# NVlabs/CenterPose

Hardware: NVIDIA H100
Metric: images/sec at 512x512 DLA-34 (dla_34 + DCNv2, 7 heads, decode + PnP) (higher is better)
Workload: dtype tf32x3

## Files before the change

centerpose_b200/csrc/conv_tma.cu:

```cuda
#include <cuda.h>

#include "common.cuh"
#include "umma_common.cuh"

namespace cp {
namespace {

constexpr int TM_BM = 128;
constexpr int TM_THREADS = 384;
constexpr int TM_THREADS_X3 = 512;

struct TmaConvParams {
  CUtensorMap amap[4];
  int nsrc;
  int srcC[4];
  int B, H, W, Cin, Cout, CoutPad, BN;
  int k;
  int tile_m;
  int Wt, boxh;
  int tiles_per_image;
  long long total_tiles;
  long long m_tiles;
  uint32_t slab_bytes, slab_stride;
  int SA, SB;
// ... 156 lines not shown
          if constexpr (MULTI) {
            const TileGeo g = decode_tile<MULTI>(p, tile / KS_SPLIT, n_tiles);
            wsrc = p.wtiles + (size_t)g.model * p.tstride +
                   ((size_t)g.n_tile * KB_all + (size_t)(tile % KS_SPLIT) * KB) * btile_bytes;
          } else {
            const int n_tile = (int)((tile / KS_SPLIT) % n_tiles);
            wsrc = p.wtiles + ((size_t)n_tile * KB_all + (size_t)(tile % KS_SPLIT) * KB) * btile_bytes;
          }
          for (int kb = 0; kb < KB; ++kb) {
            mbar_wait(smem_u32(&ctl->b_empty[stage]), phase ^ 1u);
            const uint32_t bar = smem_u32(&ctl->b_full[stage]);
            mbar_arrive_expect_tx(bar, btile_bytes);
            bulk_g2s(btiles0 + (uint32_t)stage * btile_bytes, wsrc + (size_t)kb * btile_bytes, btile_bytes, bar);
            if (++stage == p.SB) {
              stage = 0;
              phase ^= 1u;
            }
          }
        }
      }
      __syncwarp();
    }
  } else if (X3 && warp >= 12) {
    asm volatile("setmaxnreg.dec.sync.aligned.u32 48;");
    const int st = tid - 384;
    int stage = 0;
    uint32_t phase = 0;
    const uint32_t nchunk = p.slab_bytes >> 4;
    for (long long it = 0, tile = tile_at(0); tile < total_tiles; tile = tile_at(++it)) {
      for (int s = 0; s < sps; ++s) {
        mbar_wait(smem_u32(&ctl->a_full[stage]), phase);
        const uint32_t hi = slabs0 + (uint32_t)stage * a_stage;
        const uint32_t lo = hi + p.slab_stride;
        for (uint32_t c0 = st; c0 < nchunk; c0 += 128 * 4) {
          float4 v[4];
#pragma unroll
          for (int u = 0; u < 4; ++u)
            if (c0 + u * 128 < nchunk) v[u] = ld_shared_v4f(hi + ((c0 + u * 128) << 4));
#pragma unroll
          for (int u = 0; u < 4; ++u) {
            if (c0 + u * 128 < nchunk) {
              float4 h, l;
              h.x = tf32_round(v[u].x); l.x = tf32_round(v[u].x - h.x);
              h.y = tf32_round(v[u].y); l.y = tf32_round(v[u].y - h.y);
              h.z = tf32_round(v[u].z); l.z = tf32_round(v[u].z - h.z);
              h.w = tf32_round(v[u].w); l.w = tf32_round(v[u].w - h.w);
              st_shared_v4f(hi + ((c0 + u * 128) << 4), h.x, h.y, h.z, h.w);
              st_shared_v4f(lo + ((c0 + u * 128) << 4), l.x, l.y, l.z, l.w);
            }
          }
        }
        fence_proxy_async_smem();
        mbar_arrive(smem_u32(&ctl->a_split[stage]));
        if (++stage == p.SA) {
          stage = 0;
          phase ^= 1u;
        }
      }
    }
  } else {
    if (X3) asm volatile("setmaxnreg.inc.sync.aligned.u32 208;");
    const int c = (warp - 4) >> 2, wt = tid & 127;
    float* dstage = reinterpret_cast<float*>(smem + (drain0 - smem_u32(smem))) + (size_t)c * (DRAIN_STAGE_BYTES / 4);
    const uint32_t bar_a = smem_u32(X3 ? &ctl->a_split[0] : &ctl->a_full[0]);
    const uint32_t bar_a_empty = smem_u32(&ctl->a_empty[0]);
    const uint32_t bar_b_full = smem_u32(&ctl->b_full[0]), bar_b_empty = smem_u32(&ctl->b_empty[0]);
    const uint32_t a_lo_u = p.slab_stride >> 4, b_lo_u = ((uint32_t)BN * rowb) >> 4;
    EpiParams ep;
    ep.bias = p.bias;
    ep.residual = p.residual;
    ep.resStride = p.resStride;
    ep.relu = p.relu;
    ep.res_after_relu = p.res_after_relu;
    ep.round_tf32 = p.round_tf32;
    ep.out = p.out;
    ep.outStride = p.outStride;
    ep.out_nchw = p.out_nchw;
    ep.Cout = p.Cout;
    ep.CoutPad = p.CoutPad;
    ep.H = p.H;
    ep.W = p.W;
    int sa = 0, sb = 0;
    uint32_t pa = 0, pb = 0;
    float acc[BN / 2];
    float sums[X3 ? BN / 2 : 1];
    float acc2[FUSE ? 16 : 1];
#pragma unroll
    for (int j = 0; j < BN / 2; ++j) acc[j] = 0.f;
#pragma unroll
    for (int j = 0; j < (FUSE ? 16 : 1); ++j) acc2[j] = 0.f;
    for (long long it = 0, tile = tile_at(0); tile < total_tiles; tile = tile_at(++it)) {
      const TileGeo g = decode_tile<MULTI>(p, tile / KS_SPLIT, n_tiles);
      const uint32_t row0 = (p.k == 3 ? (uint32_t)(g.g0 - 1 - g.r_lo * p.Wt) : 0u) + (uint32_t)c * 64u;
#pragma unroll
      for (int j = 0; j < (X3 ? BN / 2 : 1); ++j) sums[j] = 0.f;
      int kbi = 0, gk = 0;
      for (int s = 0; s < sps; ++s) {
        mbar_wait(bar_a + 8u * (uint32_t)sa, pa);
        const uint32_t a_slab = slabs0 + (uint32_t)sa * a_stage;
        for (int tap = 0; tap < taps; ++tap, ++kbi) {
          const int ky = tap / 3, kx = tap - ky * 3;
          const uint32_t arow = row0 + (p.k == 3 ? (uint32_t)(ky * p.Wt + kx) : 0u);
          mbar_wait(bar_b_full + 8u * (uint32_t)sb, pb);
          const uint64_t da = make_desc(a_slab + arow * rowb, p.cslab);
          const uint64_t db = make_desc(btiles0 + (uint32_t)sb * btile_bytes, p.cslab);
          const bool fresh = X3 ? gk == 0 : kbi == 0;
          if (p.cslab == 32)
            mma_kblock<BN, X3, false, 4>(acc, da, db, a_lo_u, b_lo_u, fresh);
          else
            mma_kblock<BN, X3, false, 2>(acc, da, db, a_lo_u, b_lo_u, fresh);
          if (wt == 0) {
            mbar_arrive(bar_b_empty + 8u * (uint32_t)sb);
            if (tap == taps - 1) mbar_arrive(bar_a_empty + 8u * (uint32_t)sa);
          }
          if (++sb == p.SB) {
            sb = 0;
            pb ^= 1u;
          }
          if (X3) {
            if (gk == p.group - 1 || kbi == KB - 1) {
#pragma unroll
              for (int j = 0; j < (X3 ? BN / 2 : 1); ++j) sums[j] += acc[X3 ? j : 0];
              gk = 0;
            } else {
              ++gk;
            }
          }
        }
        if (++sa == p.SA) {
          sa = 0;
          pa ^= 1u;
        }
      }
      const int r_me = wt >> 1;
      int n, oy, ox, m;
      const bool valid = tile_position<MULTI>(p, g, c * 64 + r_me, &n, &oy, &ox, &m);
      const int col_end = min(p.Cout, (g.n_tile + 1) * BN);
      const int head = FUSE ? g.n_tile / p.tph : 0, part = FUSE ? g.n_tile - head * p.tph : 0;
      const size_t wofs = MULTI ? (size_t)g.model * p.wstride : 0;
      if (MULTI) ep.bias = p.bias + wofs;
      if (FUSE && part == 0) {
#pragma unroll
        for (int j = 0; j < (FUSE ? 16 : 1); ++j) acc2[j] = 0.f;
      }
      auto fn = [&](int r, int cb, float (&v)[16]) {
        if (cb >= BN) return;
        if (!FUSE && KS_SPLIT > 1) {
          const long long mn = tile / KS_SPLIT;
          const int ks = (int)(tile % KS_SPLIT);
          float4* mine = reinterpret_cast<float4*>(p.part) + (((size_t)mn * KS_SPLIT + ks) * (BN >> 2) + (cb >> 2)) * p.tile_m +
                         c * 64 + r;
#pragma unroll
          for (int q = 0; q < 4; ++q) __stcg(mine + (size_t)q * p.tile_m, make_float4(v[4 * q], v[4 * q + 1], v[4 * q + 2], v[4 * q + 3]));
        } else if (FUSE) {
          const float* b1 = p.bias + wofs + (size_t)g.n_tile * BN + cb;
          const float4* w2 = reinterpret_cast<const float4*>(p.fuse_w[head] + wofs) + ((size_t)part * BN + cb) * 4;
#pragma unroll
          for (int q = 0; q < 16; ++q) {
            const float h = fmaxf(v[q] + __ldg(b1 + q), 0.f);
#pragma unroll
            for (int u = 0; u < 4; ++u) {
              const float4 w = __ldg(w2 + q * 4 + u);
              acc2[FUSE ? 4 * u + 0 : 0] = fmaf(h, w.x, acc2[FUSE ? 4 * u + 0 : 0]);
              acc2[FUSE ? 4 * u + 1 : 0] = fmaf(h, w.y, acc2[FUSE ? 4 * u + 1 : 0]);
              acc2[FUSE ? 4 * u + 2 : 0] = fmaf(h, w.z, acc2[FUSE ? 4 * u + 2 : 0]);
              acc2[FUSE ? 4 * u + 3 : 0] = fmaf(h, w.w, acc2[FUSE ? 4 * u + 3 : 0]);
            }
          }
        } else {
          epilogue_row<16>(ep, v, valid, m, n, oy, ox, g.n_tile * BN + cb, col_end);
        }
      };
      if constexpr (X3)
        drain_rows<BN>(sums, dstage, wt, 1 + c, fn);
      else
        drain_rows<BN>(acc, dstage, wt, 1 + c, fn);
      if (FUSE && part == p.tph - 1) {
#pragma unroll
        for (int j = 0; j < (FUSE ? 16 : 1); ++j) acc2[j] += __shfl_xor_sync(0xffffffffu, acc2[j], 1);
        if ((wt & 1) == 0 && valid) {
          const int co = p.fuse_cout[head];
          float* o = p.fuse_out[head] + ((size_t)n * co * p.H + oy) * p.W + ox;
          const size_t plane = (size_t)p.H * p.W;
#pragma unroll
          for (int j = 0; j < 16; ++j)
            if (j < co) o[j * plane] = acc2[FUSE ? j : 0] + __ldg(p.fuse_b[head] + wofs + j);
        }
      }
    }
  }
}

__global__ void pack_tma_weight_kernel(const float* __restrict__ src, int ld, int Cin, int taps, int Cout, int BN, int n_tiles,
                                       int round_tf32, int x3, int cslab, unsigned char* __restrict__ dst) {
  const int KB = (Cin / cslab) * taps;
  const int cpr = cslab / 4;
  const size_t rowb = (size_t)cslab * 4;
  const size_t total = (size_t)n_tiles * KB * BN * cpr;
  for (size_t i = blockIdx.x * (size_t)blockDim.x + threadIdx.x; i < total; i += (size_t)gridDim.x * blockDim.x) {
    const int q = i % cpr;
    size_t t = i / cpr;
    const int nr = t % BN;
    t /= BN;
    const int kb = t % KB;
    const int nt = t / KB;
    const int n = nt * BN + nr;
    const int slab = kb / taps, tap = kb - slab * taps;
    float v[4];
#pragma unroll
    for (int j = 0; j < 4; ++j) {
      const int k = tap * Cin + slab * cslab + q * 4 + j;
      float x = (n < Cout) ? src[(size_t)k * ld + n] : 0.f;
      v[j] = round_tf32 ? tf32_round(x) : x;
    }
    const size_t tile = ((size_t)nt * KB + kb) * (size_t)BN * rowb * (x3 ? 2 : 1);
    const int sw = cslab == 32 ? (nr & 7) : ((nr >> 1) & 3);
    const size_t off = (size_t)nr * rowb + (size_t)((q ^ sw) << 4);
    *reinterpret_cast<float4*>(dst + tile + off) = make_float4(v[0], v[1], v[2], v[3]);
    if (x3) {
      float l[4];
#pragma unroll
      for (int j = 0; j < 4; ++j) {
        const int k = tap * Cin + slab * cslab + q * 4 + j;
        const float x = (n < Cout) ? src[(size_t)k * ld + n] : 0.f;
        l[j] = tf32_round(x - v[j]);
      }
      *reinterpret_cast<float4*>(dst + tile + (size_t)BN * rowb + off) = make_float4(l[0], l[1], l[2], l[3]);
    }
  }
}

typedef CUresult (*EncodeTiledFn)(CUtensorMap*, CUtensorMapDataType, cuuint32_t, void*, const cuuint64_t*, const cuuint64_t*,
                                  const cuuint32_t*, const cuuint32_t*, CUtensorMapInterleave, CUtensorMapSwizzle,
                                  CUtensorMapL2promotion, CUtensorMapFloatOOBfill);

EncodeTiledFn get_encode() {
  static EncodeTiledFn fn = nullptr;
  if (!fn) {
    void* p = nullptr;
    cudaDriverEntryPointQueryResult q;
    if (cudaGetDriverEntryPoint("cuTensorMapEncodeTiled", &p, cudaEnableDefault, &q) == cudaSuccess &&
        q == cudaDriverEntryPointSuccess)
      fn = (EncodeTiledFn)p;
  }
  return fn;
}

}

template <bool MULTI>
__global__ void __launch_bounds__(256) conv_tma_splitk_finish(const __grid_constant__ TmaConvParams p, long long mn_tiles) {
  splitk_finish<MULTI>(p, p.tile_m, mn_tiles, [&](long long mn, int i, int* n, int* oy, int* ox) {
    int m;
    return tile_position<MULTI>(p, decode_tile<MULTI>(p, mn, p.CoutPad / p.BN), i, n, oy, ox, &m);
  });
}

static int tma_boxh(int Wt) { return (TM_BM + 1 + 2 * Wt + Wt - 1) / Wt + 1; }

// ... 35 lines not shown
  if (p.mode != IGEMM_NHWC_VEC) return false;
  if (!((p.kh == 1 && p.kw == 1 && p.pad == 0) || (p.kh == 3 && p.kw == 3 && p.pad == 1))) return false;
  if (p.stride != 1) return false;
  const int cs = tma_cslab(p, x3);
  if (p.Cin % cs) return false;
  for (int s = 0; s < p.nsrc; ++s)
    if (p.srcC[s] % cs || p.srcStride[s] % 4) return false;
  if (p.kh == 3 && p.Win + 2 > 256) return false;
  const int bn = tma_tile_n(p.CoutPad, x3);
  if (bn == 0) return false;
  const size_t slab = p.kh == 3 ? (size_t)tma_boxh(p.Win + 2) * (p.Win + 2) * cs * 4 : (size_t)TM_BM * cs * 4;
  const size_t a_stage = ((slab + 1023) / 1024 * 1024) * (x3 ? 2 : 1);
  const size_t btile = (size_t)bn * cs * 4 * (x3 ? 2 : 1);
  if (a_stage + 2 * btile > TM_BUDGET) return false;
  return get_encode() != nullptr;
}

size_t tma_weight_bytes(int Cin, int taps, int CoutPad, int x3) {
  return (size_t)CoutPad * Cin * taps * 4 * (x3 ? 2 : 1);
}

int launch_pack_tma_weight(const float* src, int ld, int Cin, int taps, int Cout, int CoutPad, int x3, int cs, int bn,
                           void* dst, cudaStream_t s) {
  const int nt = CoutPad / bn;
  size_t total = (size_t)nt * (Cin / cs) * taps * bn * (cs / 4);
  int blocks = (int)((total + 255) / 256);
  if (blocks > 132 * 32) blocks = 132 * 32;
  pack_tma_weight_kernel<<<blocks, 256, 0, s>>>(src, ld, Cin, taps, Cout, bn, nt, 1, x3, cs, (unsigned char*)dst);
  CP_LAUNCH_CHECK("pack_tma_weight_kernel");
  return CP_OK;
}

int tma_encode_nhwc_box(const float* base, int C, int W, int H, int B, int strideFloats, int boxC, int boxW, int boxH,
                        int swizzle64, void* map_out) {
  EncodeTiledFn enc = get_encode();
  if (!enc) return fail(CP_ERR_CUDA, "cuTensorMapEncodeTiled entry point not available");
  cuuint64_t dims[4] = {(cuuint64_t)C, (cuuint64_t)W, (cuuint64_t)H, (cuuint64_t)B};
  cuuint64_t strides[3] = {(cuuint64_t)strideFloats * 4, (cuuint64_t)W * strideFloats * 4, (cuuint64_t)H * W * strideFloats * 4};
  cuuint32_t box[4] = {(cuuint32_t)boxC, (cuuint32_t)boxW, (cuuint32_t)boxH, 1};
  cuuint32_t es[4] = {1, 1, 1, 1};
  CUresult r = enc(reinterpret_cast<CUtensorMap*>(map_out), CU_TENSOR_MAP_DATA_TYPE_FLOAT32, 4, (void*)base, dims, strides, box,
                   es, CU_TENSOR_MAP_INTERLEAVE_NONE, swizzle64 ? CU_TENSOR_MAP_SWIZZLE_64B : CU_TENSOR_MAP_SWIZZLE_NONE,
                   CU_TENSOR_MAP_L2_PROMOTION_L2_256B,
                   CU_TENSOR_MAP_FLOAT_OOB_FILL_NONE);
  if (r != CUDA_SUCCESS) return fail(CP_ERR_CUDA, "cuTensorMapEncodeTiled failed with code " + std::to_string((int)r));
  return CP_OK;
}

int tma_conv_encode(const IgemmParams& p, int Bmax, int cs, void* maps_out) {
  EncodeTiledFn enc = get_encode();
  if (!enc) return fail(CP_ERR_CUDA, "cuTensorMapEncodeTiled entry point not available");
  CUtensorMap* maps = reinterpret_cast<CUtensorMap*>(maps_out);
  const int Wt = p.Win + 2;
  const int boxh = tma_boxh(Wt);
  const CUtensorMapSwizzle swz = cs == 32 ? CU_TENSOR_MAP_SWIZZLE_128B : CU_TENSOR_MAP_SWIZZLE_64B;
  for (int s = 0; s < p.nsrc; ++s) {
    CUresult r;
    if (p.kh == 3) {
      cuuint64_t dims[4] = {(cuuint64_t)p.srcC[s], (cuuint64_t)p.Win, (cuuint64_t)p.Hin, (cuuint64_t)Bmax};
      cuuint64_t strides[3] = {(cuuint64_t)p.srcStride[s] * 4, (cuuint64_t)p.Win * p.srcStride[s] * 4,
                               (cuuint64_t)p.Hin * p.Win * p.srcStride[s] * 4};
      cuuint32_t box[4] = {(cuuint32_t)cs, (cuuint32_t)Wt, (cuuint32_t)boxh, 1};
      cuuint32_t es[4] = {1, 1, 1, 1};
      r = enc(&maps[s], CU_TENSOR_MAP_DATA_TYPE_FLOAT32, 4, (void*)p.src[s], dims, strides, box, es,
              CU_TENSOR_MAP_INTERLEAVE_NONE, swz, CU_TENSOR_MAP_L2_PROMOTION_L2_256B,
              CU_TENSOR_MAP_FLOAT_OOB_FILL_NONE);
    } else {
      cuuint64_t dims[2] = {(cuuint64_t)p.srcC[s], (cuuint64_t)Bmax * p.Hin * p.Win};
      cuuint64_t strides[1] = {(cuuint64_t)p.srcStride[s] * 4};
      cuuint32_t box[2] = {(cuuint32_t)cs, (cuuint32_t)TM_BM};
      cuuint32_t es[2] = {1, 1};
      r = enc(&maps[s], CU_TENSOR_MAP_DATA_TYPE_FLOAT32, 2, (void*)p.src[s], dims, strides, box, es,
              CU_TENSOR_MAP_INTERLEAVE_NONE, swz, CU_TENSOR_MAP_L2_PROMOTION_L2_256B,
              CU_TENSOR_MAP_FLOAT_OOB_FILL_NONE);
    }
    if (r != CUDA_SUCCESS) return fail(CP_ERR_CUDA, "cuTensorMapEncodeTiled failed with code " + std::to_string((int)r));
  }
  return CP_OK;
}

template <bool X3, bool FUSE, bool MULTI>
static int launch_conv_tma_kernel(const TmaConvParams& q, const cudaLaunchConfig_t& cfg0) {
  void (*kern)(TmaConvParams) = nullptr;
  switch (q.BN) {
    case 16: kern = conv_tma_kernel<X3, FUSE, 16, MULTI>; break;
    case 32: kern = conv_tma_kernel<X3, FUSE, 32, MULTI>; break;
    case 64: kern = conv_tma_kernel<X3, FUSE, 64, MULTI>; break;
    case 128: kern = conv_tma_kernel<X3, FUSE, 128, MULTI>; break;
    default: return fail(CP_ERR_INVALID, "conv_tma: unsupported N tile");
  }
  static PerDevice<bool, 4> configured;
  const int slot = q.BN == 128 ? 3 : (q.BN == 64 ? 2 : (q.BN == 32 ? 1 : 0));
  if (!configured.here(slot)) {
    CP_CUDA_CHECK(cudaFuncSetAttribute(kern, cudaFuncAttributeMaxDynamicSharedMemorySize, 227 * 1024));
    configured.here(slot) = true;
  }
  cudaLaunchConfig_t cfg = cfg0;
  cudaLaunchAttribute attr[1];
  attr[0].id = cudaLaunchAttributeProgrammaticStreamSerialization;
  attr[0].val.programmaticStreamSerializationAllowed = 1;
  cfg.attrs = attr;
  cfg.numAttrs = g_pdl ? 1 : 0;
  CP_CUDA_CHECK(cudaLaunchKernelEx(&cfg, kern, q));
  CP_LAUNCH_CHECK("conv_tma_kernel");
  return CP_OK;
}

int launch_conv_tma(const IgemmParams& p, const void* maps, const ConvKernel& k, cudaStream_t stream, LaunchInfo* info) {
  if (!p.wgt_umma) return fail(CP_ERR_INVALID, "conv_tma: weight tiles missing");
  if (p.B % model_ipm(p)) return fail(CP_ERR_INVALID, "conv_tma: batch is not a whole number of models");
  const bool x3 = k.x3;
  TmaConvParams q;
  memset(&q, 0, sizeof(q));
  memcpy(q.amap, maps, sizeof(CUtensorMap) * 4);
  q.nsrc = p.nsrc;
  for (int s = 0; s < 4; ++s) q.srcC[s] = p.srcC[s];
  q.B = p.B;
  q.H = p.Hin;
  q.W = p.Win;
  q.Cin = p.Cin;
  q.Cout = p.Cout;
  q.CoutPad = p.CoutPad;
  q.BN = k.BN;
  q.x3 = x3;
  q.cslab = k.cslab;
  q.group = kX3GroupBlocks * (32 / q.cslab);
  q.k = p.kh;
  q.Wt = p.Win + 2;
  q.tile_m = TM_BM;
  q.boxh = tma_boxh(q.Wt);
  q.ipm = model_ipm(p);
  q.wstride = p.wstride;
  q.tstride = p.tstride;
  size_t m_tiles;
  if (q.k == 3) {
    q.tiles_per_image = (p.Hin * q.Wt + q.tile_m - 1) / q.tile_m;
    m_tiles = (size_t)q.tiles_per_image * p.B;
    q.slab_bytes = (uint32_t)q.boxh * q.Wt * (uint32_t)q.cslab * 4u;
  } else {
    q.tiles_per_image = 0;
    q.tiles_per_model = ((long long)q.ipm * p.Hin * p.Win + q.tile_m - 1) / q.tile_m;
    m_tiles = (size_t)q.tiles_per_model * (p.B / q.ipm);
    q.slab_bytes = (uint32_t)q.tile_m * (uint32_t)q.cslab * 4u;
  }
  q.slab_stride = (q.slab_bytes + 1023u) & ~1023u;
  const uint32_t btile = (uint32_t)q.BN * (uint32_t)q.cslab * 4u * (x3 ? 2u : 1u);
  const uint32_t a_stage = q.slab_stride * (x3 ? 2u : 1u);
  size_t smem = 0;
  if (int rc = tma_smem_layout(a_stage, btile, q.k, &q.SA, &q.SB, &smem)) return rc;
  q.bias = p.bias;
  q.residual = p.residual;
  q.resStride = p.resStride;
  q.relu = p.relu;
  q.res_after_relu = p.res_after_relu;
  q.out = p.out;
  q.outStride = p.outStride;
  q.out_nchw = p.out_nchw;
  q.round_tf32 = k.round_out;
  q.wtiles = (const unsigned char*)p.wgt_umma;
  if (p.fuse_n > 0) {
    if (p.fuse_hidden % q.BN || p.CoutPad != p.fuse_n * p.fuse_hidden || !p.relu || p.residual || (x3 && q.BN != 128))
      return fail(CP_ERR_INVALID, "conv_tma: fused 1x1 needs relu, no residual and head_conv a multiple of the N tile");
    q.fuse = 1;
    q.tph = p.fuse_hidden / q.BN;
    for (int h = 0; h < p.fuse_n; ++h) {
      q.fuse_w[h] = p.fuse_w[h];
      q.fuse_b[h] = p.fuse_b[h];
      q.fuse_out[h] = p.fuse_out[h];
      q.fuse_cout[h] = p.fuse_cout[h];
    }
  }
  q.m_tiles = (long long)m_tiles;
  q.part = p.splitk_ws;
// ... 38 lines not shown
```

centerpose_b200/csrc/umma_common.cuh:

```cuda
#pragma once
#include <cuda.h>
#include <cuda_runtime.h>
#include <stdint.h>
#include <stdio.h>

namespace cp {
namespace umma {

__device__ __forceinline__ uint32_t smem_u32(const void* p) { return (uint32_t)__cvta_generic_to_shared(p); }

__device__ __forceinline__ void mbar_init(uint32_t bar, uint32_t count) {
  asm volatile("mbarrier.init.shared::cta.b64 [%0], %1;" ::"r"(bar), "r"(count));
}
__device__ __forceinline__ void mbar_arrive(uint32_t bar) {
  asm volatile("mbarrier.arrive.shared::cta.b64 _, [%0];" ::"r"(bar) : "memory");
}
__device__ __forceinline__ void mbar_arrive_expect_tx(uint32_t bar, uint32_t bytes) {
  asm volatile("mbarrier.arrive.expect_tx.shared::cta.b64 _, [%0], %1;" ::"r"(bar), "r"(bytes) : "memory");
}
__device__ __forceinline__ bool mbar_try_wait(uint32_t bar, uint32_t parity) {
  uint32_t ok;
  asm volatile(
      "{\n\t.reg .pred p;\n\tmbarrier.try_wait.parity.shared::cta.b64 p, [%1], %2;\n\tselp.b32 %0, 1, 0, p;\n\t}"
      : "=r"(ok)
// ... 54 lines not shown
}
template <> __device__ __forceinline__ void wgmma_tf32<128>(float (&d)[64], uint64_t da, uint64_t db, uint32_t scale_d) {
  asm volatile(
      "{\n\t.reg .pred p;\n\tsetp.ne.b32 p, %66, 0;\n\t"
      "wgmma.mma_async.sync.aligned.m64n128k8.f32.tf32.tf32 {%0,%1,%2,%3,%4,%5,%6,%7,%8,%9,%10,%11,%12,%13,%14,%15,%16,%17,%18,%19,%20,%21,%22,%23,%24,%25,%26,%27,%28,%29,%30,%31,%32,%33,%34,%35,%36,%37,%38,%39,%40,%41,%42,%43,%44,%45,%46,%47,%48,%49,%50,%51,%52,%53,%54,%55,%56,%57,%58,%59,%60,%61,%62,%63}, %64, %65, p, 1, 1;\n\t}"
      : "+f"(d[0]), "+f"(d[1]), "+f"(d[2]), "+f"(d[3]), "+f"(d[4]), "+f"(d[5]), "+f"(d[6]), "+f"(d[7]), "+f"(d[8]), "+f"(d[9]), "+f"(d[10]), "+f"(d[11]), "+f"(d[12]), "+f"(d[13]), "+f"(d[14]), "+f"(d[15]), "+f"(d[16]), "+f"(d[17]), "+f"(d[18]), "+f"(d[19]), "+f"(d[20]), "+f"(d[21]), "+f"(d[22]), "+f"(d[23]), "+f"(d[24]), "+f"(d[25]), "+f"(d[26]), "+f"(d[27]), "+f"(d[28]), "+f"(d[29]), "+f"(d[30]), "+f"(d[31]), "+f"(d[32]), "+f"(d[33]), "+f"(d[34]), "+f"(d[35]), "+f"(d[36]), "+f"(d[37]), "+f"(d[38]), "+f"(d[39]), "+f"(d[40]), "+f"(d[41]), "+f"(d[42]), "+f"(d[43]), "+f"(d[44]), "+f"(d[45]), "+f"(d[46]), "+f"(d[47]), "+f"(d[48]), "+f"(d[49]), "+f"(d[50]), "+f"(d[51]), "+f"(d[52]), "+f"(d[53]), "+f"(d[54]), "+f"(d[55]), "+f"(d[56]), "+f"(d[57]), "+f"(d[58]), "+f"(d[59]), "+f"(d[60]), "+f"(d[61]), "+f"(d[62]), "+f"(d[63])
      : "l"(da), "l"(db), "r"(scale_d));
}
template <> __device__ __forceinline__ void wgmma_tf32<256>(float (&d)[128], uint64_t da, uint64_t db, uint32_t scale_d) {
  asm volatile(
      "{\n\t.reg .pred p;\n\tsetp.ne.b32 p, %130, 0;\n\t"
      "wgmma.mma_async.sync.aligned.m64n256k8.f32.tf32.tf32 {%0,%1,%2,%3,%4,%5,%6,%7,%8,%9,%10,%11,%12,%13,%14,%15,%16,%17,%18,%19,%20,%21,%22,%23,%24,%25,%26,%27,%28,%29,%30,%31,%32,%33,%34,%35,%36,%37,%38,%39,%40,%41,%42,%43,%44,%45,%46,%47,%48,%49,%50,%51,%52,%53,%54,%55,%56,%57,%58,%59,%60,%61,%62,%63,%64,%65,%66,%67,%68,%69,%70,%71,%72,%73,%74,%75,%76,%77,%78,%79,%80,%81,%82,%83,%84,%85,%86,%87,%88,%89,%90,%91,%92,%93,%94,%95,%96,%97,%98,%99,%100,%101,%102,%103,%104,%105,%106,%107,%108,%109,%110,%111,%112,%113,%114,%115,%116,%117,%118,%119,%120,%121,%122,%123,%124,%125,%126,%127}, %128, %129, p, 1, 1;\n\t}"
      : "+f"(d[0]), "+f"(d[1]), "+f"(d[2]), "+f"(d[3]), "+f"(d[4]), "+f"(d[5]), "+f"(d[6]), "+f"(d[7]), "+f"(d[8]), "+f"(d[9]), "+f"(d[10]), "+f"(d[11]), "+f"(d[12]), "+f"(d[13]), "+f"(d[14]), "+f"(d[15]), "+f"(d[16]), "+f"(d[17]), "+f"(d[18]), "+f"(d[19]), "+f"(d[20]), "+f"(d[21]), "+f"(d[22]), "+f"(d[23]), "+f"(d[24]), "+f"(d[25]), "+f"(d[26]), "+f"(d[27]), "+f"(d[28]), "+f"(d[29]), "+f"(d[30]), "+f"(d[31]), "+f"(d[32]), "+f"(d[33]), "+f"(d[34]), "+f"(d[35]), "+f"(d[36]), "+f"(d[37]), "+f"(d[38]), "+f"(d[39]), "+f"(d[40]), "+f"(d[41]), "+f"(d[42]), "+f"(d[43]), "+f"(d[44]), "+f"(d[45]), "+f"(d[46]), "+f"(d[47]), "+f"(d[48]), "+f"(d[49]), "+f"(d[50]), "+f"(d[51]), "+f"(d[52]), "+f"(d[53]), "+f"(d[54]), "+f"(d[55]), "+f"(d[56]), "+f"(d[57]), "+f"(d[58]), "+f"(d[59]), "+f"(d[60]), "+f"(d[61]), "+f"(d[62]), "+f"(d[63]), "+f"(d[64]), "+f"(d[65]), "+f"(d[66]), "+f"(d[67]), "+f"(d[68]), "+f"(d[69]), "+f"(d[70]), "+f"(d[71]), "+f"(d[72]), "+f"(d[73]), "+f"(d[74]), "+f"(d[75]), "+f"(d[76]), "+f"(d[77]), "+f"(d[78]), "+f"(d[79]), "+f"(d[80]), "+f"(d[81]), "+f"(d[82]), "+f"(d[83]), "+f"(d[84]), "+f"(d[85]), "+f"(d[86]), "+f"(d[87]), "+f"(d[88]), "+f"(d[89]), "+f"(d[90]), "+f"(d[91]), "+f"(d[92]), "+f"(d[93]), "+f"(d[94]), "+f"(d[95]), "+f"(d[96]), "+f"(d[97]), "+f"(d[98]), "+f"(d[99]), "+f"(d[100]), "+f"(d[101]), "+f"(d[102]), "+f"(d[103]), "+f"(d[104]), "+f"(d[105]), "+f"(d[106]), "+f"(d[107]), "+f"(d[108]), "+f"(d[109]), "+f"(d[110]), "+f"(d[111]), "+f"(d[112]), "+f"(d[113]), "+f"(d[114]), "+f"(d[115]), "+f"(d[116]), "+f"(d[117]), "+f"(d[118]), "+f"(d[119]), "+f"(d[120]), "+f"(d[121]), "+f"(d[122]), "+f"(d[123]), "+f"(d[124]), "+f"(d[125]), "+f"(d[126]), "+f"(d[127])
      : "l"(da), "l"(db), "r"(scale_d));
}
template <> __device__ __forceinline__ void wgmma_bf16<16>(float (&d)[8], uint64_t da, uint64_t db, uint32_t scale_d) {
  asm volatile(
      "{\n\t.reg .pred p;\n\tsetp.ne.b32 p, %10, 0;\n\t"
      "wgmma.mma_async.sync.aligned.m64n16k16.f32.bf16.bf16 {%0,%1,%2,%3,%4,%5,%6,%7}, %8, %9, p, 1, 1, 0, 0;\n\t}"
      : "+f"(d[0]), "+f"(d[1]), "+f"(d[2]), "+f"(d[3]), "+f"(d[4]), "+f"(d[5]), "+f"(d[6]), "+f"(d[7])
      : "l"(da), "l"(db), "r"(scale_d));
}
template <> __device__ __forceinline__ void wgmma_bf16<32>(float (&d)[16], uint64_t da, uint64_t db, uint32_t scale_d) {
  asm volatile(
      "{\n\t.reg .pred p;\n\tsetp.ne.b32 p, %18, 0;\n\t"
      "wgmma.mma_async.sync.aligned.m64n32k16.f32.bf16.bf16 {%0,%1,%2,%3,%4,%5,%6,%7,%8,%9,%10,%11,%12,%13,%14,%15}, %16, %17, p, 1, 1, 0, 0;\n\t}"
      : "+f"(d[0]), "+f"(d[1]), "+f"(d[2]), "+f"(d[3]), "+f"(d[4]), "+f"(d[5]), "+f"(d[6]), "+f"(d[7]), "+f"(d[8]), "+f"(d[9]), "+f"(d[10]), "+f"(d[11]), "+f"(d[12]), "+f"(d[13]), "+f"(d[14]), "+f"(d[15])
      : "l"(da), "l"(db), "r"(scale_d));
}
template <> __device__ __forceinline__ void wgmma_bf16<64>(float (&d)[32], uint64_t da, uint64_t db, uint32_t scale_d) {
  asm volatile(
      "{\n\t.reg .pred p;\n\tsetp.ne.b32 p, %34, 0;\n\t"
      "wgmma.mma_async.sync.aligned.m64n64k16.f32.bf16.bf16 {%0,%1,%2,%3,%4,%5,%6,%7,%8,%9,%10,%11,%12,%13,%14,%15,%16,%17,%18,%19,%20,%21,%22,%23,%24,%25,%26,%27,%28,%29,%30,%31}, %32, %33, p, 1, 1, 0, 0;\n\t}"
      : "+f"(d[0]), "+f"(d[1]), "+f"(d[2]), "+f"(d[3]), "+f"(d[4]), "+f"(d[5]), "+f"(d[6]), "+f"(d[7]), "+f"(d[8]), "+f"(d[9]), "+f"(d[10]), "+f"(d[11]), "+f"(d[12]), "+f"(d[13]), "+f"(d[14]), "+f"(d[15]), "+f"(d[16]), "+f"(d[17]), "+f"(d[18]), "+f"(d[19]), "+f"(d[20]), "+f"(d[21]), "+f"(d[22]), "+f"(d[23]), "+f"(d[24]), "+f"(d[25]), "+f"(d[26]), "+f"(d[27]), "+f"(d[28]), "+f"(d[29]), "+f"(d[30]), "+f"(d[31])
      : "l"(da), "l"(db), "r"(scale_d));
}
template <> __device__ __forceinline__ void wgmma_bf16<128>(float (&d)[64], uint64_t da, uint64_t db, uint32_t scale_d) {
  asm volatile(
      "{\n\t.reg .pred p;\n\tsetp.ne.b32 p, %66, 0;\n\t"
      "wgmma.mma_async.sync.aligned.m64n128k16.f32.bf16.bf16 {%0,%1,%2,%3,%4,%5,%6,%7,%8,%9,%10,%11,%12,%13,%14,%15,%16,%17,%18,%19,%20,%21,%22,%23,%24,%25,%26,%27,%28,%29,%30,%31,%32,%33,%34,%35,%36,%37,%38,%39,%40,%41,%42,%43,%44,%45,%46,%47,%48,%49,%50,%51,%52,%53,%54,%55,%56,%57,%58,%59,%60,%61,%62,%63}, %64, %65, p, 1, 1, 0, 0;\n\t}"
      : "+f"(d[0]), "+f"(d[1]), "+f"(d[2]), "+f"(d[3]), "+f"(d[4]), "+f"(d[5]), "+f"(d[6]), "+f"(d[7]), "+f"(d[8]), "+f"(d[9]), "+f"(d[10]), "+f"(d[11]), "+f"(d[12]), "+f"(d[13]), "+f"(d[14]), "+f"(d[15]), "+f"(d[16]), "+f"(d[17]), "+f"(d[18]), "+f"(d[19]), "+f"(d[20]), "+f"(d[21]), "+f"(d[22]), "+f"(d[23]), "+f"(d[24]), "+f"(d[25]), "+f"(d[26]), "+f"(d[27]), "+f"(d[28]), "+f"(d[29]), "+f"(d[30]), "+f"(d[31]), "+f"(d[32]), "+f"(d[33]), "+f"(d[34]), "+f"(d[35]), "+f"(d[36]), "+f"(d[37]), "+f"(d[38]), "+f"(d[39]), "+f"(d[40]), "+f"(d[41]), "+f"(d[42]), "+f"(d[43]), "+f"(d[44]), "+f"(d[45]), "+f"(d[46]), "+f"(d[47]), "+f"(d[48]), "+f"(d[49]), "+f"(d[50]), "+f"(d[51]), "+f"(d[52]), "+f"(d[53]), "+f"(d[54]), "+f"(d[55]), "+f"(d[56]), "+f"(d[57]), "+f"(d[58]), "+f"(d[59]), "+f"(d[60]), "+f"(d[61]), "+f"(d[62]), "+f"(d[63])
      : "l"(da), "l"(db), "r"(scale_d));
}
template <> __device__ __forceinline__ void wgmma_bf16<256>(float (&d)[128], uint64_t da, uint64_t db, uint32_t scale_d) {
  asm volatile(
      "{\n\t.reg .pred p;\n\tsetp.ne.b32 p, %130, 0;\n\t"
      "wgmma.mma_async.sync.aligned.m64n256k16.f32.bf16.bf16 {%0,%1,%2,%3,%4,%5,%6,%7,%8,%9,%10,%11,%12,%13,%14,%15,%16,%17,%18,%19,%20,%21,%22,%23,%24,%25,%26,%27,%28,%29,%30,%31,%32,%33,%34,%35,%36,%37,%38,%39,%40,%41,%42,%43,%44,%45,%46,%47,%48,%49,%50,%51,%52,%53,%54,%55,%56,%57,%58,%59,%60,%61,%62,%63,%64,%65,%66,%67,%68,%69,%70,%71,%72,%73,%74,%75,%76,%77,%78,%79,%80,%81,%82,%83,%84,%85,%86,%87,%88,%89,%90,%91,%92,%93,%94,%95,%96,%97,%98,%99,%100,%101,%102,%103,%104,%105,%106,%107,%108,%109,%110,%111,%112,%113,%114,%115,%116,%117,%118,%119,%120,%121,%122,%123,%124,%125,%126,%127}, %128, %129, p, 1, 1, 0, 0;\n\t}"
      : "+f"(d[0]), "+f"(d[1]), "+f"(d[2]), "+f"(d[3]), "+f"(d[4]), "+f"(d[5]), "+f"(d[6]), "+f"(d[7]), "+f"(d[8]), "+f"(d[9]), "+f"(d[10]), "+f"(d[11]), "+f"(d[12]), "+f"(d[13]), "+f"(d[14]), "+f"(d[15]), "+f"(d[16]), "+f"(d[17]), "+f"(d[18]), "+f"(d[19]), "+f"(d[20]), "+f"(d[21]), "+f"(d[22]), "+f"(d[23]), "+f"(d[24]), "+f"(d[25]), "+f"(d[26]), "+f"(d[27]), "+f"(d[28]), "+f"(d[29]), "+f"(d[30]), "+f"(d[31]), "+f"(d[32]), "+f"(d[33]), "+f"(d[34]), "+f"(d[35]), "+f"(d[36]), "+f"(d[37]), "+f"(d[38]), "+f"(d[39]), "+f"(d[40]), "+f"(d[41]), "+f"(d[42]), "+f"(d[43]), "+f"(d[44]), "+f"(d[45]), "+f"(d[46]), "+f"(d[47]), "+f"(d[48]), "+f"(d[49]), "+f"(d[50]), "+f"(d[51]), "+f"(d[52]), "+f"(d[53]), "+f"(d[54]), "+f"(d[55]), "+f"(d[56]), "+f"(d[57]), "+f"(d[58]), "+f"(d[59]), "+f"(d[60]), "+f"(d[61]), "+f"(d[62]), "+f"(d[63]), "+f"(d[64]), "+f"(d[65]), "+f"(d[66]), "+f"(d[67]), "+f"(d[68]), "+f"(d[69]), "+f"(d[70]), "+f"(d[71]), "+f"(d[72]), "+f"(d[73]), "+f"(d[74]), "+f"(d[75]), "+f"(d[76]), "+f"(d[77]), "+f"(d[78]), "+f"(d[79]), "+f"(d[80]), "+f"(d[81]), "+f"(d[82]), "+f"(d[83]), "+f"(d[84]), "+f"(d[85]), "+f"(d[86]), "+f"(d[87]), "+f"(d[88]), "+f"(d[89]), "+f"(d[90]), "+f"(d[91]), "+f"(d[92]), "+f"(d[93]), "+f"(d[94]), "+f"(d[95]), "+f"(d[96]), "+f"(d[97]), "+f"(d[98]), "+f"(d[99]), "+f"(d[100]), "+f"(d[101]), "+f"(d[102]), "+f"(d[103]), "+f"(d[104]), "+f"(d[105]), "+f"(d[106]), "+f"(d[107]), "+f"(d[108]), "+f"(d[109]), "+f"(d[110]), "+f"(d[111]), "+f"(d[112]), "+f"(d[113]), "+f"(d[114]), "+f"(d[115]), "+f"(d[116]), "+f"(d[117]), "+f"(d[118]), "+f"(d[119]), "+f"(d[120]), "+f"(d[121]), "+f"(d[122]), "+f"(d[123]), "+f"(d[124]), "+f"(d[125]), "+f"(d[126]), "+f"(d[127])
      : "l"(da), "l"(db), "r"(scale_d));
}

template <int N>
__device__ __forceinline__ void wgmma_tf32_rs(float (&d)[N / 2], const uint32_t (&a)[4], uint64_t db, uint32_t scale_d);
template <> __device__ __forceinline__ void wgmma_tf32_rs<16>(float (&d)[8], const uint32_t (&a)[4], uint64_t db, uint32_t scale_d) {
  asm volatile(
      "{\n\t.reg .pred p;\n\tsetp.ne.b32 p, %13, 0;\n\t"
      "wgmma.mma_async.sync.aligned.m64n16k8.f32.tf32.tf32 {%0,%1,%2,%3,%4,%5,%6,%7}, {%8,%9,%10,%11}, %12, p, 1, 1;\n\t}"
      : "+f"(d[0]), "+f"(d[1]), "+f"(d[2]), "+f"(d[3]), "+f"(d[4]), "+f"(d[5]), "+f"(d[6]), "+f"(d[7])
      : "r"(a[0]), "r"(a[1]), "r"(a[2]), "r"(a[3]), "l"(db), "r"(scale_d));
}
template <> __device__ __forceinline__ void wgmma_tf32_rs<32>(float (&d)[16], const uint32_t (&a)[4], uint64_t db, uint32_t scale_d) {
  asm volatile(
      "{\n\t.reg .pred p;\n\tsetp.ne.b32 p, %21, 0;\n\t"
      "wgmma.mma_async.sync.aligned.m64n32k8.f32.tf32.tf32 {%0,%1,%2,%3,%4,%5,%6,%7,%8,%9,%10,%11,%12,%13,%14,%15}, {%16,%17,%18,%19}, %20, p, 1, 1;\n\t}"
      : "+f"(d[0]), "+f"(d[1]), "+f"(d[2]), "+f"(d[3]), "+f"(d[4]), "+f"(d[5]), "+f"(d[6]), "+f"(d[7]), "+f"(d[8]), "+f"(d[9]), "+f"(d[10]), "+f"(d[11]), "+f"(d[12]), "+f"(d[13]), "+f"(d[14]), "+f"(d[15])
      : "r"(a[0]), "r"(a[1]), "r"(a[2]), "r"(a[3]), "l"(db), "r"(scale_d));
}
template <> __device__ __forceinline__ void wgmma_tf32_rs<64>(float (&d)[32], const uint32_t (&a)[4], uint64_t db, uint32_t scale_d) {
  asm volatile(
      "{\n\t.reg .pred p;\n\tsetp.ne.b32 p, %37, 0;\n\t"
      "wgmma.mma_async.sync.aligned.m64n64k8.f32.tf32.tf32 {%0,%1,%2,%3,%4,%5,%6,%7,%8,%9,%10,%11,%12,%13,%14,%15,%16,%17,%18,%19,%20,%21,%22,%23,%24,%25,%26,%27,%28,%29,%30,%31}, {%32,%33,%34,%35}, %36, p, 1, 1;\n\t}"
      : "+f"(d[0]), "+f"(d[1]), "+f"(d[2]), "+f"(d[3]), "+f"(d[4]), "+f"(d[5]), "+f"(d[6]), "+f"(d[7]), "+f"(d[8]), "+f"(d[9]), "+f"(d[10]), "+f"(d[11]), "+f"(d[12]), "+f"(d[13]), "+f"(d[14]), "+f"(d[15]), "+f"(d[16]), "+f"(d[17]), "+f"(d[18]), "+f"(d[19]), "+f"(d[20]), "+f"(d[21]), "+f"(d[22]), "+f"(d[23]), "+f"(d[24]), "+f"(d[25]), "+f"(d[26]), "+f"(d[27]), "+f"(d[28]), "+f"(d[29]), "+f"(d[30]), "+f"(d[31])
      : "r"(a[0]), "r"(a[1]), "r"(a[2]), "r"(a[3]), "l"(db), "r"(scale_d));
}
template <> __device__ __forceinline__ void wgmma_tf32_rs<128>(float (&d)[64], const uint32_t (&a)[4], uint64_t db, uint32_t scale_d) {
  asm volatile(
      "{\n\t.reg .pred p;\n\tsetp.ne.b32 p, %69, 0;\n\t"
      "wgmma.mma_async.sync.aligned.m64n128k8.f32.tf32.tf32 {%0,%1,%2,%3,%4,%5,%6,%7,%8,%9,%10,%11,%12,%13,%14,%15,%16,%17,%18,%19,%20,%21,%22,%23,%24,%25,%26,%27,%28,%29,%30,%31,%32,%33,%34,%35,%36,%37,%38,%39,%40,%41,%42,%43,%44,%45,%46,%47,%48,%49,%50,%51,%52,%53,%54,%55,%56,%57,%58,%59,%60,%61,%62,%63}, {%64,%65,%66,%67}, %68, p, 1, 1;\n\t}"
      : "+f"(d[0]), "+f"(d[1]), "+f"(d[2]), "+f"(d[3]), "+f"(d[4]), "+f"(d[5]), "+f"(d[6]), "+f"(d[7]), "+f"(d[8]), "+f"(d[9]), "+f"(d[10]), "+f"(d[11]), "+f"(d[12]), "+f"(d[13]), "+f"(d[14]), "+f"(d[15]), "+f"(d[16]), "+f"(d[17]), "+f"(d[18]), "+f"(d[19]), "+f"(d[20]), "+f"(d[21]), "+f"(d[22]), "+f"(d[23]), "+f"(d[24]), "+f"(d[25]), "+f"(d[26]), "+f"(d[27]), "+f"(d[28]), "+f"(d[29]), "+f"(d[30]), "+f"(d[31]), "+f"(d[32]), "+f"(d[33]), "+f"(d[34]), "+f"(d[35]), "+f"(d[36]), "+f"(d[37]), "+f"(d[38]), "+f"(d[39]), "+f"(d[40]), "+f"(d[41]), "+f"(d[42]), "+f"(d[43]), "+f"(d[44]), "+f"(d[45]), "+f"(d[46]), "+f"(d[47]), "+f"(d[48]), "+f"(d[49]), "+f"(d[50]), "+f"(d[51]), "+f"(d[52]), "+f"(d[53]), "+f"(d[54]), "+f"(d[55]), "+f"(d[56]), "+f"(d[57]), "+f"(d[58]), "+f"(d[59]), "+f"(d[60]), "+f"(d[61]), "+f"(d[62]), "+f"(d[63])
      : "r"(a[0]), "r"(a[1]), "r"(a[2]), "r"(a[3]), "l"(db), "r"(scale_d));
}

template <int BN, bool X3, bool BF16, int KS>
__device__ __forceinline__ void mma_kblock(float (&acc)[BN / 2], uint64_t da, uint64_t db, uint32_t a_lo, uint32_t b_lo,
                                           bool fresh) {
  wg_fence();
#pragma unroll
  for (int ks = 0; ks < KS; ++ks) {
    const uint32_t sd = (fresh && ks == 0) ? 0u : 1u;
    if (X3) {
      wgmma_tf32<BN>(acc, da + a_lo + 2u * ks, db + 2u * ks, sd);
      wgmma_tf32<BN>(acc, da + 2u * ks, db + b_lo + 2u * ks, 1u);
    } else if (BF16) {
      wgmma_bf16<BN>(acc, da + 2u * ks, db + 2u * ks, sd);
    } else {
      wgmma_tf32<BN>(acc, da + 2u * ks, db + 2u * ks, sd);
    }
  }
  if (X3) {
#pragma unroll
    for (int ks = 0; ks < KS; ++ks) wgmma_tf32<BN>(acc, da + 2u * ks, db + 2u * ks, 1u);
  }
  wg_commit();
  wg_wait<0>();
}

__device__ __forceinline__ float tf32_round(float x) {
  return __uint_as_float((__float_as_uint(x) + 0x1000u) & 0xffffe000u);
}
__device__ __forceinline__ void ldsm_x4(uint32_t (&r)[4], uint32_t addr) {
  asm volatile("ldmatrix.sync.aligned.m8n8.x4.shared.b16 {%0, %1, %2, %3}, [%4];"
               : "=r"(r[0]), "=r"(r[1]), "=r"(r[2]), "=r"(r[3])
               : "r"(addr));
}

template <int BN, int KS>
__device__ __forceinline__ void mma_kblock_x3(float (&acc)[BN / 2], uint32_t a_tile, int wt, uint64_t db, uint32_t b_lo,
                                              bool fresh) {
  const uint32_t lane = (uint32_t)wt & 31u;
  const uint32_t row = (uint32_t)(wt >> 5) * 16u + (lane & 7u) + ((lane >> 3) & 1u) * 8u;
  const uint32_t a_row = a_tile + row * (32u * KS);
  const uint32_t x = ((lane >> 4) << 4) ^ ((a_row >> 3) & (KS == 4 ? 0x70u : 0x30u));
  uint32_t hi[KS][4], lo[KS][4];
#pragma unroll
  for (int ks = 0; ks < KS; ++ks) {
    ldsm_x4(hi[ks], a_row + (((uint32_t)ks << 5) ^ x));
#pragma unroll
    for (int j = 0; j < 4; ++j) {
      const float v = __uint_as_float(hi[ks][j]);
      const float h = tf32_round(v);
      lo[ks][j] = __float_as_uint(tf32_round(v - h));
      hi[ks][j] = __float_as_uint(h);
    }
  }
  wg_fence();
#pragma unroll
  for (int ks = 0; ks < KS; ++ks) {
    wgmma_tf32_rs<BN>(acc, lo[ks], db + 2u * ks, (fresh && ks == 0) ? 0u : 1u);
    wgmma_tf32_rs<BN>(acc, hi[ks], db + b_lo + 2u * ks, 1u);
  }
#pragma unroll
  for (int ks = 0; ks < KS; ++ks) wgmma_tf32_rs<BN>(acc, hi[ks], db + 2u * ks, 1u);
  wg_commit();
  wg_wait<0>();
#pragma unroll
  for (int ks = 0; ks < KS; ++ks)
#pragma unroll
    for (int j = 0; j < 4; ++j) asm volatile("" : "+r"(hi[ks][j]), "+r"(lo[ks][j]));
}

__device__ __forceinline__ uint32_t pack_bf16x2(float a, float b) {
  uint32_t r;
  asm("cvt.rn.bf16x2.f32 %0, %1, %2;" : "=r"(r) : "f"(b), "f"(a));
  return r;
}
__device__ __forceinline__ void st_shared_v4(uint32_t addr, uint32_t a, uint32_t b, uint32_t c, uint32_t d) {
  asm volatile("st.shared.v4.b32 [%0], {%1, %2, %3, %4};" ::"r"(addr), "r"(a), "r"(b), "r"(c), "r"(d) : "memory");
}
__device__ __forceinline__ void st_shared_v4f(uint32_t addr, float a, float b, float c, float d) {
  asm volatile("st.shared.v4.f32 [%0], {%1, %2, %3, %4};" ::"r"(addr), "f"(a), "f"(b), "f"(c), "f"(d) : "memory");
}
__device__ __forceinline__ float4 ld_shared_v4f(uint32_t addr) {
  float4 v;
  asm volatile("ld.shared.v4.f32 {%0,%1,%2,%3}, [%4];" : "=f"(v.x), "=f"(v.y), "=f"(v.z), "=f"(v.w) : "r"(addr) : "memory");
  return v;
}

__device__ __forceinline__ void tma_load_4d(uint32_t dst, const CUtensorMap* map, int c0, int c1, int c2, int c3, uint32_t bar) {
  asm volatile(
      "cp.async.bulk.tensor.4d.shared::cluster.global.tile.mbarrier::complete_tx::bytes [%0], [%1, {%2, %3, %4, %5}], [%6];" ::"r"(dst),
      "l"(map), "r"(c0), "r"(c1), "r"(c2), "r"(c3), "r"(bar)
      : "memory");
}
__device__ __forceinline__ void tma_load_2d(uint32_t dst, const CUtensorMap* map, int c0, int c1, uint32_t bar) {
  asm volatile("cp.async.bulk.tensor.2d.shared::cluster.global.tile.mbarrier::complete_tx::bytes [%0], [%1, {%2, %3}], [%4];" ::"r"(dst),
               "l"(map), "r"(c0), "r"(c1), "r"(bar)
               : "memory");
}
__device__ __forceinline__ bool elect_one() {
  uint32_t pred;
  asm volatile("{\n\t.reg .pred p;\n\telect.sync _|p, 0xffffffff;\n\tselp.u32 %0, 1, 0, p;\n\t}" : "=r"(pred));
  return pred != 0;
}

__device__ __forceinline__ uint64_t make_desc(uint32_t saddr, int cslab) {
  const uint64_t sbo = cslab == 32 ? (1024 >> 4) : (512 >> 4);
// ... 122 lines not shown
```

Measured before the change: 678.4.

## Overlap WGMMA k-blocks with async wait and ping-pong accumulators in TMA conv

Splits the k-block MMA helper into an issue step and a separate wait, so the conv consumer loop keeps one WGMMA group in flight (wait<1>) while it acquires and issues the next one. Buffer release to the producer is deferred until the prior group retires. For the X3 path with BN<=64, two accumulator sets alternate per group so the promotion into the running sums overlaps the next group's MMAs. BN=128 X3 issues two k-blocks before waiting. The X3+FUSE launch is restricted to BN=128, and the delayed-release logic adds register pressure and complexity around barrier ordering.

```diff
diff --git a/centerpose_b200/csrc/conv_tma.cu b/centerpose_b200/csrc/conv_tma.cu
--- a/centerpose_b200/csrc/conv_tma.cu
+++ b/centerpose_b200/csrc/conv_tma.cu
@@ -262,54 +262,146 @@
     ep.W = p.W;
     int sa = 0, sb = 0;
     uint32_t pa = 0, pb = 0;
-    float acc[BN / 2];
+    constexpr bool PINGPONG = X3 && BN <= 64;
+    float acc[PINGPONG ? 2 : 1][BN / 2];
     float sums[X3 ? BN / 2 : 1];
     float acc2[FUSE ? 16 : 1];
 #pragma unroll
-    for (int j = 0; j < BN / 2; ++j) acc[j] = 0.f;
+    for (int a = 0; a < (PINGPONG ? 2 : 1); ++a)
+#pragma unroll
+      for (int j = 0; j < BN / 2; ++j) acc[a][j] = 0.f;
 #pragma unroll
     for (int j = 0; j < (FUSE ? 16 : 1); ++j) acc2[j] = 0.f;
+    struct KBlock {
+      uint64_t da, db;
+      int sa, sb;
+      bool slab_end, fresh, group_end;
+    };
+    auto release = [&](const KBlock& k) {
+      if (wt == 0) {
+        mbar_arrive(bar_b_empty + 8u * (uint32_t)k.sb);
+        if (k.slab_end) mbar_arrive(bar_a_empty + 8u * (uint32_t)k.sa);
+      }
+    };
+    auto issue = [&](float (&a)[BN / 2], uint64_t da, uint64_t db, bool fresh) {
+      if (p.cslab == 32)
+        mma_kblock_issue<BN, X3, false, 4>(a, da, db, a_lo_u, b_lo_u, fresh);
+      else
+        mma_kblock_issue<BN, X3, false, 2>(a, da, db, a_lo_u, b_lo_u, fresh);
+    };
+    auto promote = [&](const float (&a)[BN / 2]) {
+#pragma unroll
+      for (int j = 0; j < BN / 2; ++j) sums[X3 ? j : 0] += a[j];
+    };
     for (long long it = 0, tile = tile_at(0); tile < total_tiles; tile = tile_at(++it)) {
       const TileGeo g = decode_tile<MULTI>(p, tile / KS_SPLIT, n_tiles);
       const uint32_t row0 = (p.k == 3 ? (uint32_t)(g.g0 - 1 - g.r_lo * p.Wt) : 0u) + (uint32_t)c * 64u;
 #pragma unroll
       for (int j = 0; j < (X3 ? BN / 2 : 1); ++j) sums[j] = 0.f;
-      int kbi = 0, gk = 0;
-      for (int s = 0; s < sps; ++s) {
-        mbar_wait(bar_a + 8u * (uint32_t)sa, pa);
-        const uint32_t a_slab = slabs0 + (uint32_t)sa * a_stage;
-        for (int tap = 0; tap < taps; ++tap, ++kbi) {
-          const int ky = tap / 3, kx = tap - ky * 3;
-          const uint32_t arow = row0 + (p.k == 3 ? (uint32_t)(ky * p.Wt + kx) : 0u);
-          mbar_wait(bar_b_full + 8u * (uint32_t)sb, pb);
-          const uint64_t da = make_desc(a_slab + arow * rowb, p.cslab);
-          const uint64_t db = make_desc(btiles0 + (uint32_t)sb * btile_bytes, p.cslab);
-          const bool fresh = X3 ? gk == 0 : kbi == 0;
-          if (p.cslab == 32)
-            mma_kblock<BN, X3, false, 4>(acc, da, db, a_lo_u, b_lo_u, fresh);
-          else
-            mma_kblock<BN, X3, false, 2>(acc, da, db, a_lo_u, b_lo_u, fresh);
-          if (wt == 0) {
-            mbar_arrive(bar_b_empty + 8u * (uint32_t)sb);
-            if (tap == taps - 1) mbar_arrive(bar_a_empty + 8u * (uint32_t)sa);
+      int kbi = 0, gk = 0, tap = 0;
+      auto acquire = [&](auto&& drain) {
+        if (tap == 0) {
+          if (p.SA == 1) drain();
+          mbar_wait(bar_a + 8u * (uint32_t)sa, pa);
+        }
+        const int ky = tap / 3, kx = tap - ky * 3;
+        const uint32_t arow = row0 + (p.k == 3 ? (uint32_t)(ky * p.Wt + kx) : 0u);
+        mbar_wait(bar_b_full + 8u * (uint32_t)sb, pb);
+        KBlock k;
+        k.da = make_desc(slabs0 + (uint32_t)sa * a_stage + arow * rowb, p.cslab);
+        k.db = make_desc(btiles0 + (uint32_t)sb * btile_bytes, p.cslab);
+        k.sa = sa;
+        k.sb = sb;
+        k.slab_end = tap == taps - 1;
+        k.fresh = X3 ? gk == 0 : kbi == 0;
+        k.group_end = gk == p.group - 1 || kbi == KB - 1;
+        gk = k.group_end ? 0 : gk + 1;
+        ++kbi;
+        if (++sb == p.SB) {
+          sb = 0;
+          pb ^= 1u;
+        }
+        if (++tap == taps) {
+          tap = 0;
+          if (++sa == p.SA) {
+            sa = 0;
+            pa ^= 1u;
           }
-          if (++sb == p.SB) {
-            sb = 0;
-            pb ^= 1u;
+        }
+        return k;
+      };
+      KBlock prev{};
+      bool pend = false;
+      if constexpr (!X3) {
+        auto retire = [&]() {
+          if (pend) release(prev);
+          pend = false;
+        };
+        auto drain = [&]() {
+          wg_wait<0>();
+          retire();
+        };
+        while (kbi < KB) {
+          const KBlock k = acquire(drain);
+          issue(acc[0], k.da, k.db, k.fresh);
+          wg_wait<1>();
+          retire();
+          prev = k;
+          pend = true;
+        }
+        drain();
+      } else if constexpr (PINGPONG) {
+        auto run_group = [&](float (&a)[BN / 2], float (&o)[BN / 2]) {
+          auto retire = [&]() {
+            if (pend) {
+              if (prev.group_end) promote(o);
+              release(prev);
+            }
+            pend = false;
+          };
+          auto kblock = [&]() {
+            const KBlock k = acquire([&]() {
+              wg_wait<0>();
+              retire();
+            });
+            issue(a, k.da, k.db, k.fresh);
+            wg_wait<1>();
+            retire();
+            prev = k;
+            pend = true;
+          };
+          kblock();
+          if (!prev.group_end) kblock();
+        };
+        while (kbi < KB) {
+          run_group(acc[0], acc[1]);
+          if (kbi < KB) run_group(acc[1], acc[0]);
+        }
+        wg_wait<0>();
+        if (((KB + p.group - 1) / p.group) & 1)
+          promote(acc[0]);
+        else
+          promote(acc[PINGPONG ? 1 : 0]);
+        release(prev);
+      } else {
+        while (kbi < KB) {
+          KBlock k = acquire([]() {});
+          issue(acc[0], k.da, k.db, k.fresh);
+          if (!k.group_end) {
+            prev = k;
+            k = acquire([&]() {
+              wg_wait<0>();
+              release(prev);
+              prev.sb = -1;
+            });
+            issue(acc[0], k.da, k.db, k.fresh);
+          } else {
+            prev.sb = -1;
           }
-          if (X3) {
-            if (gk == p.group - 1 || kbi == KB - 1) {
-#pragma unroll
-              for (int j = 0; j < (X3 ? BN / 2 : 1); ++j) sums[j] += acc[X3 ? j : 0];
-              gk = 0;
-            } else {
-              ++gk;
-            }
-          }
-        }
-        if (++sa == p.SA) {
-          sa = 0;
-          pa ^= 1u;
+          wg_wait<0>();
+          if (prev.sb >= 0) release(prev);
+          release(k);
+          promote(acc[0]);
         }
       }
       const int r_me = wt >> 1;
@@ -354,7 +446,7 @@
       if constexpr (X3)
         drain_rows<BN>(sums, dstage, wt, 1 + c, fn);
       else
-        drain_rows<BN>(acc, dstage, wt, 1 + c, fn);
+        drain_rows<BN>(acc[0], dstage, wt, 1 + c, fn);
       if (FUSE && part == p.tph - 1) {
 #pragma unroll
         for (int j = 0; j < (FUSE ? 16 : 1); ++j) acc2[j] += __shfl_xor_sync(0xffffffffu, acc2[j], 1);
@@ -556,13 +648,17 @@
 template <bool X3, bool FUSE, bool MULTI>
 static int launch_conv_tma_kernel(const TmaConvParams& q, const cudaLaunchConfig_t& cfg0) {
   void (*kern)(TmaConvParams) = nullptr;
-  switch (q.BN) {
-    case 16: kern = conv_tma_kernel<X3, FUSE, 16, MULTI>; break;
-    case 32: kern = conv_tma_kernel<X3, FUSE, 32, MULTI>; break;
-    case 64: kern = conv_tma_kernel<X3, FUSE, 64, MULTI>; break;
-    case 128: kern = conv_tma_kernel<X3, FUSE, 128, MULTI>; break;
-    default: return fail(CP_ERR_INVALID, "conv_tma: unsupported N tile");
-  }
+  if constexpr (X3 && FUSE) {
+    if (q.BN == 128) kern = conv_tma_kernel<X3, FUSE, 128, MULTI>;
+  } else {
+    switch (q.BN) {
+      case 16: kern = conv_tma_kernel<X3, FUSE, 16, MULTI>; break;
+      case 32: kern = conv_tma_kernel<X3, FUSE, 32, MULTI>; break;
+      case 64: kern = conv_tma_kernel<X3, FUSE, 64, MULTI>; break;
+      case 128: kern = conv_tma_kernel<X3, FUSE, 128, MULTI>; break;
+    }
+  }
+  if (!kern) return fail(CP_ERR_INVALID, "conv_tma: unsupported N tile");
   static PerDevice<bool, 4> configured;
   const int slot = q.BN == 128 ? 3 : (q.BN == 64 ? 2 : (q.BN == 32 ? 1 : 0));
   if (!configured.here(slot)) {
diff --git a/centerpose_b200/csrc/umma_common.cuh b/centerpose_b200/csrc/umma_common.cuh
--- a/centerpose_b200/csrc/umma_common.cuh
+++ b/centerpose_b200/csrc/umma_common.cuh
@@ -160,8 +160,8 @@
 }
 
 template <int BN, bool X3, bool BF16, int KS>
-__device__ __forceinline__ void mma_kblock(float (&acc)[BN / 2], uint64_t da, uint64_t db, uint32_t a_lo, uint32_t b_lo,
-                                           bool fresh) {
+__device__ __forceinline__ void mma_kblock_issue(float (&acc)[BN / 2], uint64_t da, uint64_t db, uint32_t a_lo,
+                                                 uint32_t b_lo, bool fresh) {
   wg_fence();
 #pragma unroll
   for (int ks = 0; ks < KS; ++ks) {
@@ -180,6 +180,11 @@
     for (int ks = 0; ks < KS; ++ks) wgmma_tf32<BN>(acc, da + 2u * ks, db + 2u * ks, 1u);
   }
   wg_commit();
+}
+template <int BN, bool X3, bool BF16, int KS>
+__device__ __forceinline__ void mma_kblock(float (&acc)[BN / 2], uint64_t da, uint64_t db, uint32_t a_lo, uint32_t b_lo,
+                                           bool fresh) {
+  mma_kblock_issue<BN, X3, BF16, KS>(acc, da, db, a_lo, b_lo, fresh);
   wg_wait<0>();
 }
 
```

Measured after the change: 692.1, median of 6. +2.0%, better.
